# lixinghe1999/VRVQ

Hardware: AMD Instinct MI355X
Metric: audio-sec/s encode+RVQ+decode, 44.1 kHz batch-32, 1->8 MI355X; RVQ HBM GB/s (higher is better)
Workload: dtype f32; 1 GPU; DAC_VRVQ VBR 8 cb, level 1.0, 1-s clips, preprocess+encode+decode (z_q_is materialised); model=DAC_VRVQ base (8 cb), global_batch=32, clip_samples=44100, n_codebooks=8, parallelism=dp1 (replicas, no data-path collective)

## Files before the change

vrvq_amd/csrc/conv.hip:

```cpp
#include "common.h"
#include "conv_core.h"
#include "conv_x3.h"
#include <atomic>

namespace {

using namespace vrvq_conv;

template <int BM, int BN, int WM, int NW, int KS, bool X3, bool PH = false,
          bool PAIR = x3_pair<KS, BM, BN>(), bool SPLIT = false>
__global__ __launch_bounds__(64 * NW)
__attribute__((amdgpu_waves_per_eu(X3 && x3_stages<BM, BN>() == 1 ? 2 : 1)))
void conv_mfma_kernel(ConvArgs a) {
  using TC = TileCfg<BM, BN, WM, NW>;
  extern __shared__ __attribute__((aligned(16))) float smem[];
  int bid = blockIdx.x;
  int ks = 0;
  if (SPLIT) {
    ks = bid % a.ks_split;
    bid /= a.ks_split;
  }
  const int mt = bid % a.n_mt;
  bid /= a.n_mt;
  const int nt = bid % a.n_nt;
// ... 562 lines not shown
    const int kk = (int)(rk % k);
    const int ci = (int)(rk / k);
    wp[i] = co < cout ? w[((size_t)co * cin + ci) * k + kk] : 0.0f;
  }
}

__global__ void pack_convt1d_kernel(const float* __restrict__ w, int cin, int cout, int s,
                                    int cout_pad, float* __restrict__ wp) {
  const size_t total = (size_t)cin * 2 * cout_pad;
  for (size_t i = blockIdx.x * (size_t)blockDim.x + threadIdx.x; i < total;
       i += (size_t)gridDim.x * blockDim.x) {
    const int mm = (int)(i % cout_pad);
    const size_t rk = i / cout_pad;
    const int tap = (int)(rk % 2);
    const int ci = (int)(rk / 2);
    float v = 0.0f;
    if (mm < cout * s) {
      const int co = mm / s, r = mm - co * s;
      const int kk = tap == 1 ? r : r + s;
      v = w[((size_t)ci * cout + co) * (2 * s) + kk];
    }
    wp[i] = v;
  }
}

template <int KS>
__global__ void pack_x3_kernel(const float* __restrict__ wp, int cin, int m_pad,
                               u32x4* __restrict__ w3, size_t total) {
  using XC = X3Cfg<KS>;
  for (size_t i = blockIdx.x * (size_t)blockDim.x + threadIdx.x; i < total;
       i += (size_t)gridDim.x * blockDim.x) {
    const int m = (int)(i % m_pad);
    size_t r = i / m_pad;
    const int o = (int)(r % XC::NO2);
    r /= XC::NO2;
    const int plane = (int)(r % 3);
    const int chunk = (int)(r / 3);
    const int tap = o / XC::NC8, c8 = o - tap * XC::NC8;
    float v[8];
#pragma unroll
    for (int u = 0; u < 8; ++u) {
      const int ci = chunk * XC::CK + c8 * 8 + u;
      v[u] = (o < XC::NO && ci < cin) ? wp[((size_t)ci * KS + tap) * m_pad + m] : 0.0f;
    }
    unsigned h[4], mm[4], l[4];
#pragma unroll
    for (int u = 0; u < 4; ++u) split3x2(v[2 * u], v[2 * u + 1], h[u], mm[u], l[u]);
    w3[i] = plane == 0 ? u32x4{h[0], h[1], h[2], h[3]}
          : plane == 1 ? u32x4{mm[0], mm[1], mm[2], mm[3]} : u32x4{l[0], l[1], l[2], l[3]};
  }
}

static long long x3_size_u16(int cin, int k, int m_pad) {
  auto sz = [&](int ck, int no2) {
    return (long long)((cin + ck - 1) / ck) * 3 * no2 * m_pad * 8;
  };
  switch (k) {
    case 1: return sz(X3Cfg<1>::CK, X3Cfg<1>::NO2);
    case 2: return sz(X3Cfg<2>::CK, X3Cfg<2>::NO2);
    case 3: return sz(X3Cfg<3>::CK, X3Cfg<3>::NO2);
    case 7: return sz(X3Cfg<7>::CK, X3Cfg<7>::NO2);
    default: return -1;
  }
}

}

extern "C" int vrvq_x3_weight_size(int cin, int k, int cout_pad, long long* n_u16) {
  VRVQ_CHECK_ARG(n_u16 && cin > 0 && cout_pad > 0);
  const long long n = x3_size_u16(cin, k, cout_pad);
  if (n < 0) return VRVQ_ERR_UNSUPPORTED;
  *n_u16 = n;
  return 0;
}

extern "C" int vrvq_pack_x3_weight(const float* w_packed, int cin, int k, int cout_pad,
                                   uint16_t* w_x3, vrvq_stream_t stream) {
  VRVQ_CHECK_ARG(w_packed && w_x3 && cin > 0 && cout_pad > 0);
  const long long n = x3_size_u16(cin, k, cout_pad);
  if (n < 0) return VRVQ_ERR_UNSUPPORTED;
  const size_t total = (size_t)n / 8;
  const unsigned grid = (unsigned)((total + 255) / 256 < 65536 ? (total + 255) / 256 : 65536);
  u32x4* out = reinterpret_cast<u32x4*>(w_x3);
  hipStream_t st = as_stream(stream);
  switch (k) {
    case 1: hipLaunchKernelGGL(pack_x3_kernel<1>, dim3(grid), dim3(256), 0, st, w_packed, cin, cout_pad, out, total); break;
    case 2: hipLaunchKernelGGL(pack_x3_kernel<2>, dim3(grid), dim3(256), 0, st, w_packed, cin, cout_pad, out, total); break;
    case 3: hipLaunchKernelGGL(pack_x3_kernel<3>, dim3(grid), dim3(256), 0, st, w_packed, cin, cout_pad, out, total); break;
    default: hipLaunchKernelGGL(pack_x3_kernel<7>, dim3(grid), dim3(256), 0, st, w_packed, cin, cout_pad, out, total); break;
  }
  return vrvq_launch_status();
}

extern "C" int vrvq_conv1d(const float* x, int batch, int cin, int tin, const float* alpha,
                           const float* inv_alpha, const float* w_packed,
                           const uint16_t* w_x3, int cout,
                           int cout_pad, int k, int stride, int pad, int dil, const float* bias,
                           const float* residual, int epilogue, float* y, int tout,
                           const float* alpha_out, const float* inv_alpha_out, float* y_snake,
                           vrvq_stream_t stream) {
  return vrvq_conv1d_ws(x, batch, cin, tin, alpha, inv_alpha, w_packed, w_x3, cout, cout_pad, k,
                        stride, pad, dil, bias, residual, epilogue, y, tout, alpha_out,
                        inv_alpha_out, y_snake, nullptr, 0, stream);
}

extern "C" int vrvq_conv1d_workspace(int batch, int cin, int tin, int cout, int k, int stride,
                                     int pad, int dil, int x3, long long* bytes) {
  VRVQ_CHECK_ARG(bytes && batch > 0 && cin > 0 && tin > 0 && cout > 0 && k > 0 && stride > 0 &&
                 dil > 0 && pad >= 0);
  const long long tout = ((long long)tin + 2LL * pad - (long long)dil * (k - 1) - 1) / stride + 1;
  VRVQ_CHECK_ARG(tout > 0);
  int S = 0;
  if (stride > 1) {
    if (x3 && k == 2 * stride && (stride & (stride - 1)) == 0 && pad < stride)
      S = splitk_parts(cout, cin * stride, (int)tout, 2, true, false, true);
  } else {
    S = splitk_parts(cout, cin, (int)tout, k, false, false, x3 != 0);
  }
  *bytes = (long long)splitk_bytes(S, cout, (int)tout, batch);
  return 0;
}

extern "C" int vrvq_conv_last_launch(int out[5]) {
  VRVQ_CHECK_ARG(out);
  const unsigned v = g_last_launch.load(std::memory_order_relaxed);
  out[0] = (int)(v & 511);
  out[1] = (int)(v >> 9 & 511);
  out[2] = (int)(v >> 18 & 31);
  out[3] = (int)(v >> 23 & 3);
  out[4] = (int)(v >> 25 & 127);
  return 0;
}

namespace {


bool conv1d_geometry_ok(int batch, int cin, int tin, int cout, int cout_pad, int k, int stride,
                        int pad, int dil, int tout) {
  return batch > 0 && cin > 0 && tin > 0 && cout > 0 && k > 0 && stride > 0 && dil > 0 &&
         pad >= 0 && tout > 0 && cout_pad >= cout && cout_pad % 128 == 0 &&
         tout == ((long long)tin + 2LL * pad - (long long)dil * (k - 1) - 1) / stride + 1;
}

int run_conv1d(ConvArgs a, int batch, int cin, int tin, int cout, int cout_pad, int k, int stride,
               int pad, int dil, int tout, int epilogue, void* workspace, long long ws_bytes,
               hipStream_t st, ConvPlan* plan) {
  const bool proj = a.pj_part != nullptr;
  a.cin = cin; a.tin = tin; a.M = cout; a.m_pad = cout_pad; a.cout = cout;
  a.stride = stride; a.pad = pad; a.dil = dil; a.ng = tout; a.up = 0; a.up_pad = 0;
  a.ssh = 0;
  if (stride > 1 && (stride & (stride - 1)) == 0)
    while ((1 << a.ssh) < stride) ++a.ssh;
  a.ylen = tout; a.epi = epilogue;
  if (workspace != nullptr) {
    long long need = 0;
    const int rc = vrvq_conv1d_workspace(batch, cin, tin, cout, k, stride, pad, dil,
                                         a.w3 != nullptr, &need);
    if (rc) return rc;
    VRVQ_CHECK_ARG(ws_bytes >= need);
    if (need > 0) a.ks_part = static_cast<float*>(workspace);
  }
  if (a.w3 != nullptr && stride > 1) {
    if (k != 2 * stride || a.ssh == 0 || pad >= stride) return VRVQ_ERR_UNSUPPORTED;
    a.psh = a.ssh; a.ppad = pad; a.pcin = cin; a.ptin = tin;
    a.cin = cin * stride; a.tin = tout + 1;
    a.stride = 1; a.pad = 0; a.dil = 1; a.ssh = 0;
    return dispatch_ks(2, a, batch, st, plan);
  }
  if (!proj && cout <= SMALL_COUT && stride == 1 &&
      cin * k * (cout == 1 ? 1 : SMALL_COUT) <= SMALL_WMAX)
    return launch_small(a, batch, k, st, plan);
  if (!proj && cin == 1 && k == 7 && stride == 1 && dil == 1 && !a.alpha && cout % CI1_CG == 0 &&
      tout % 4 == 0) {
    const long long nblk =
        (long long)batch * ((tout + 256 * CI1_T - 1) / (256 * CI1_T)) * (cout / CI1_CG);
    if (nblk <= 0 || nblk > 0x7fffffffLL) return VRVQ_ERR_ARG;
    if (plan) *plan = ConvPlan{PATH_CIN1, 0, 0, 0, k, 0, 0};
    return launch_kernel(conv_cin1_stream_kernel<7>, nblk, 256, 0, st, a, plan != nullptr);
  }
  return dispatch_ks(k, a, batch, st, plan);
}

int run_conv_transpose1d(ConvArgs a, int batch, int cin, int tin, int cout, int cout_pad,
                         int stride, int pad, hipStream_t st, ConvPlan* plan) {
  VRVQ_CHECK_ARG(batch > 0 && cin > 0 && tin > 0 && cout > 0 && stride > 0);
  VRVQ_CHECK_ARG(pad >= 0 && pad < stride);
  VRVQ_CHECK_ARG(cout_pad >= cout * stride && cout_pad % 64 == 0);
  a.cin = cin; a.tin = tin; a.M = cout * stride; a.m_pad = cout_pad; a.cout = cout;
  a.stride = 1; a.pad = 1; a.dil = 1; a.ng = tin + 1; a.up = stride; a.up_pad = pad;
  a.ylen = (tin - 1) * stride - 2 * pad + 2 * stride;
  a.epi = VRVQ_EPI_NONE;
  return dispatch_ks(2, a, batch, st, plan);
}

}

extern "C" int vrvq_conv1d_ws(const float* x, int batch, int cin, int tin, const float* alpha,
                              const float* inv_alpha, const float* w_packed,
                              const uint16_t* w_x3, int cout, int cout_pad, int k, int stride,
                              int pad, int dil, const float* bias, const float* residual,
                              int epilogue, float* y, int tout, const float* alpha_out,
                              const float* inv_alpha_out, float* y_snake, void* workspace,
                              long long ws_bytes, vrvq_stream_t stream) {
  VRVQ_CHECK_ARG(x && w_packed && (y || y_snake));
  VRVQ_CHECK_ARG(y_snake == nullptr || (alpha_out && inv_alpha_out));
  VRVQ_CHECK_ARG(conv1d_geometry_ok(batch, cin, tin, cout, cout_pad, k, stride, pad, dil, tout));
  VRVQ_CHECK_ARG(alpha == nullptr || inv_alpha != nullptr);
  VRVQ_CHECK_ARG(epilogue >= 0 && epilogue <= 2);
  ConvArgs a{};
  a.x = x; a.alpha = alpha; a.inv_alpha = inv_alpha; a.w = w_packed;
  a.bias = bias; a.res = residual; a.y = y;
  a.alpha_o = alpha_out; a.inv_alpha_o = inv_alpha_out; a.ys = y_snake;
  a.w3 = reinterpret_cast<const unsigned*>(w_x3);
  return run_conv1d(a, batch, cin, tin, cout, cout_pad, k, stride, pad, dil, tout, epilogue,
                    workspace, ws_bytes, as_stream(stream), nullptr);
}

extern "C" int vrvq_conv1d_proj(const float* x, int batch, int cin, int tin, const float* alpha,
                                const float* inv_alpha, const float* w_packed,
                                const uint16_t* w_x3, int cout, int cout_pad, int k, int pad,
                                int dil, const float* bias, float* y, int tout,
                                const uint16_t* w3in, int nq, float* part, void* workspace,
                                long long ws_bytes, vrvq_stream_t stream) {
  VRVQ_CHECK_ARG(x && w_packed && w3in && part);
  VRVQ_CHECK_ARG(batch > 0 && cin > 0 && tin > 0 && cout > 0 && k > 0 && dil > 0 && pad >= 0 &&
                 tout > 0 && nq > 0);
  VRVQ_CHECK_ARG(cout_pad >= cout && cout_pad % 128 == 0);
  VRVQ_CHECK_ARG(alpha == nullptr || inv_alpha != nullptr);
  VRVQ_CHECK_ARG(((uintptr_t)part & 15) == 0 && ((uintptr_t)w3in & 15) == 0);
  if (cout != 1024 || nq > 32) return VRVQ_ERR_UNSUPPORTED;
  VRVQ_CHECK_ARG(conv1d_geometry_ok(batch, cin, tin, cout, cout_pad, k, 1, pad, dil, tout));
  VRVQ_CHECK_ARG((long long)batch * tout * nq * 8 * 8 < 0x7fffffffLL);
  ConvArgs a{};
  a.x = x; a.alpha = alpha; a.inv_alpha = inv_alpha; a.w = w_packed; a.bias = bias; a.y = y;
  a.w3 = reinterpret_cast<const unsigned*>(w_x3);
  a.pj_w3 = reinterpret_cast<const unsigned*>(w3in);
  a.pj_part = part;
  a.pj_nq = nq;
  a.pj_nf = batch * tout;
  return run_conv1d(a, batch, cin, tin, cout, cout_pad, k, 1, pad, dil, tout, VRVQ_EPI_NONE,
                    workspace, ws_bytes, as_stream(stream), nullptr);
}

extern "C" int vrvq_conv_transpose1d(const float* x, int batch, int cin, int tin,
                                     const float* alpha, const float* inv_alpha,
                                     const float* w_packed, int cout, int cout_pad, int stride,
                                     const float* bias, float* y, const float* alpha_out,
                                     const float* inv_alpha_out, float* y_snake,
                                     vrvq_stream_t stream) {
  return vrvq_conv_transpose1d_pad(x, batch, cin, tin, alpha, inv_alpha, w_packed, nullptr,
                                   cout, cout_pad, stride, (stride + 1) / 2, bias, y, alpha_out,
                                   inv_alpha_out, y_snake, stream);
}

extern "C" int vrvq_conv_transpose1d_pad(const float* x, int batch, int cin, int tin,
                                         const float* alpha, const float* inv_alpha,
                                         const float* w_packed, const uint16_t* w_x3,
                                         int cout, int cout_pad,
                                         int stride, int pad, const float* bias, float* y,
                                         const float* alpha_out, const float* inv_alpha_out,
                                         float* y_snake, vrvq_stream_t stream) {
  VRVQ_CHECK_ARG(x && w_packed && (y || y_snake));
  VRVQ_CHECK_ARG(y_snake == nullptr || (alpha_out && inv_alpha_out));
  VRVQ_CHECK_ARG(alpha == nullptr || inv_alpha != nullptr);
  ConvArgs a{};
  a.x = x; a.alpha = alpha; a.inv_alpha = inv_alpha; a.w = w_packed; a.bias = bias;
  a.res = nullptr; a.y = y;
  a.alpha_o = alpha_out; a.inv_alpha_o = inv_alpha_out; a.ys = y_snake;
  a.w3 = reinterpret_cast<const unsigned*>(w_x3);
  return run_conv_transpose1d(a, batch, cin, tin, cout, cout_pad, stride, pad, as_stream(stream),
                              nullptr);
}

extern "C" int vrvq_conv_plan(int kind, int batch, int cin, int tin, int cout, int k, int stride,
                              int pad, int dil, int has_x3, int has_workspace, int out[7]) {
  VRVQ_CHECK_ARG(out && kind >= VRVQ_PLAN_CONV && kind <= VRVQ_PLAN_CONV_TRANSPOSE);
  static float present[4];
  ConvArgs a{};
  a.w3 = has_x3 ? reinterpret_cast<const unsigned*>(present) : nullptr;
  void* ws = has_workspace ? present : nullptr;
  ConvPlan p{};
  int rc;
  if (kind == VRVQ_PLAN_CONV_TRANSPOSE) {
    VRVQ_CHECK_ARG(stride > 0 && k == 2 * stride && dil == 1);
    const long long rows = (long long)cout * stride, rt = 128 % stride == 0 ? 128 : 192;
    VRVQ_CHECK_ARG(cout > 0 && rows < 0x7fffff00LL);
    rc = run_conv_transpose1d(a, batch, cin, tin, cout, (int)((rows + rt - 1) / rt * rt), stride,
                              pad, nullptr, &p);
  } else {
    VRVQ_CHECK_ARG(cout > 0 && cout < 0x7fffff00 && k > 0 && stride > 0 && dil > 0 && tin > 0 &&
                   pad >= 0);
    const long long tout = ((long long)tin + 2LL * pad - (long long)dil * (k - 1) - 1) / stride + 1;
    const int cout_pad = (cout + 127) / 128 * 128;
    VRVQ_CHECK_ARG(tout > 0 && tout <= 0x7fffffffLL);
    VRVQ_CHECK_ARG(conv1d_geometry_ok(batch, cin, tin, cout, cout_pad, k, stride, pad, dil,
                                      (int)tout));
    if (kind == VRVQ_PLAN_PROJ) {
      VRVQ_CHECK_ARG(stride == 1);
      if (cout != 1024) return VRVQ_ERR_UNSUPPORTED;
      a.pj_part = present;
    }
    rc = run_conv1d(a, batch, cin, tin, cout, cout_pad, k, stride, pad, dil, (int)tout,
                    VRVQ_EPI_NONE, ws, 0x7fffffffffffffffLL, nullptr, &p);
  }
  if (rc) return rc;
  const int v[7] = {p.BM, p.BN, p.KS, p.x3, p.S, p.path, p.WM};
  for (int i = 0; i < 7; ++i) out[i] = v[i];
  return 0;
}

extern "C" int vrvq_pack_conv1d_weight(const float* w, int cout, int cin, int k, int cout_pad,
                                       float* w_packed, vrvq_stream_t stream) {
  VRVQ_CHECK_ARG(w && w_packed && cout > 0 && cin > 0 && k > 0 && cout_pad >= cout);
  const size_t total = (size_t)cin * k * cout_pad;
  const unsigned grid = (unsigned)((total + 255) / 256 < 65536 ? (total + 255) / 256 : 65536);
  hipLaunchKernelGGL(pack_conv1d_kernel, dim3(grid), dim3(256), 0, as_stream(stream), w, cout,
                     cin, k, cout_pad, w_packed);
  return vrvq_launch_status();
}

extern "C" int vrvq_pack_convt1d_weight(const float* w, int cin, int cout, int stride,
                                        int cout_pad, float* w_packed, vrvq_stream_t stream) {
  VRVQ_CHECK_ARG(w && w_packed && cout > 0 && cin > 0 && stride > 0 && cout_pad >= cout * stride);
  const size_t total = (size_t)cin * 2 * cout_pad;
  const unsigned grid = (unsigned)((total + 255) / 256 < 65536 ? (total + 255) / 256 : 65536);
  hipLaunchKernelGGL(pack_convt1d_kernel, dim3(grid), dim3(256), 0, as_stream(stream), w, cin,
                     cout, stride, cout_pad, w_packed);
  return vrvq_launch_status();
}
```

vrvq_amd/csrc/conv_ru.hip:

```cpp
#include "common.h"
#include "conv_core.h"
#include "conv_x3.h"

namespace {

using namespace vrvq_conv;

struct RuArgs {
  ConvArgs p1;
  ConvArgs p2;
  const float* b7;
  const float* alpha2;
  const float* inv_alpha2;
  const float* w1;
  const u32x4* w1x3;
  int C;
};

template <int BM, int BN>
constexpr bool ru_p2x3() { return BM * BN * 6 <= 80 * 1024; }
template <int BM, int BN, int WM>
constexpr bool ru_p2x3h() {
  return !ru_p2x3<BM, BN>() && WM == 2 && BM % 32 == 0 && BM * BN * 5 <= 80 * 1024;
}

template <int BM, int BN, int WM, int NW, bool X3>
__global__ __launch_bounds__(64 * NW)
__attribute__((amdgpu_waves_per_eu(X3 && x3_stages<BM, BN>() == 1 ? 2 : 1)))
void ru_fused_kernel(RuArgs ra) {
  using TC = TileCfg<BM, BN, WM, NW>;
  constexpr int RM = TC::RM, RN = TC::RN, TM = TC::TM, TN = TC::TN;
  constexpr int NS = BM / 2;
  constexpr int PF = 8;
  static_assert(NS % PF == 0, "phase-2 steps per group");
  extern __shared__ __attribute__((aligned(16))) float smem[];
  const ConvArgs& a = ra.p1;
  const int nt = blockIdx.x % a.n_nt;
  const int b = blockIdx.x / a.n_nt;
  const int n0 = nt * BN;
  const int C = ra.C;

  f32x16 acc[RM][RN];
#pragma unroll
  for (int i = 0; i < RM; ++i)
#pragma unroll
    for (int j = 0; j < RN; ++j)
#pragma unroll
      for (int r = 0; r < 16; ++r) acc[i][j][r] = 0.0f;
#ifdef VRVQ_X3_SB_ALL
  constexpr bool SB = true;
#else
  constexpr bool SB = BM == 96 || BM == 192 || BM == 128;
#endif
  if constexpr (X3) conv_mainloop_x3<BM, BN, WM, NW, 7, false, x3_pair<7, BM, BN>(), SB>(a, smem, acc, b, 0, n0);
  else conv_mainloop<BM, BN, WM, NW, 7>(a, smem, acc, b, 0, n0);

  const int tid = threadIdx.x, lane = tid & 63, wave = tid >> 6;
  const int wm = wave % WM, wn = wave / WM;
  const int lr = lane & 31, lh = lane >> 5;

  if constexpr (X3 && ru_p2x3<BM, BN>()) {
    if (ra.w1x3 != nullptr) {
      constexpr int NC8 = BM / 8;
      char* hsb = reinterpret_cast<char*>(smem);
#pragma unroll
      for (int i = 0; i < RM; ++i)
#pragma unroll
        for (int g = 0; g < 4; ++g) {
          const int row0 = wm * TM + i * 32 + 8 * g + 4 * lh;
          float bb[4], al[4], ia[4];
#pragma unroll
          for (int u = 0; u < 4; ++u) {
            const bool ok = row0 + u < C;
            bb[u] = ok ? ra.b7[row0 + u] : 0.0f;
            al[u] = ok ? ra.alpha2[row0 + u] : 0.0f;
            ia[u] = ok ? ra.inv_alpha2[row0 + u] : 0.0f;
          }
          const int c8 = (wm * TM + i * 32 + 8 * g) / 8;
#pragma unroll
          for (int j = 0; j < RN; ++j) {
            float v[4];
#pragma unroll
            for (int u = 0; u < 4; ++u) v[u] = acc[i][j][4 * g + u] + bb[u];
            snake_n<4>(v, al, ia);
#pragma unroll
            for (int u = 0; u < 4; ++u) v[u] = row0 + u < C ? v[u] : 0.0f;
            unsigned h[2], m[2], l[2];
            split3x2(v[0], v[1], h[0], m[0], l[0]);
            split3x2(v[2], v[3], h[1], m[1], l[1]);
            const int col = wn * TN + j * 32 + lr;
            const size_t off = ((size_t)c8 * BN + col) * 16 + lh * 8;
            typedef unsigned u32x2 __attribute__((ext_vector_type(2)));
            *reinterpret_cast<u32x2*>(hsb + off) = u32x2{h[0], h[1]};
            *reinterpret_cast<u32x2*>(hsb + (size_t)NC8 * BN * 16 + off) = u32x2{m[0], m[1]};
            *reinterpret_cast<u32x2*>(hsb + 2 * (size_t)NC8 * BN * 16 + off) = u32x2{l[0], l[1]};
          }
        }
      __syncthreads();
#pragma unroll
      for (int i = 0; i < RM; ++i)
#pragma unroll
        for (int j = 0; j < RN; ++j)
#pragma unroll
          for (int r = 0; r < 16; ++r) acc[i][j][r] = 0.0f;
      constexpr int NQ = BM / 16;
      const u32x4* hs = reinterpret_cast<const u32x4*>(hsb);
      auto lda = [&](int q, u32x4 (&av)[3][RM]) {
        const int o = 2 * q + lh;
        const int ch = o >> 2, oo = o & 3;
#pragma unroll
        for (int p = 0; p < 3; ++p)
#pragma unroll
          for (int i = 0; i < RM; ++i)
            av[p][i] = ra.w1x3[((size_t)(ch * 3 + p) * 4 + oo) * a.m_pad + wm * TM + i * 32 + lr];
      };
      u32x4 an[3][RM];
      lda(0, an);
#pragma unroll 2
      for (int q = 0; q < NQ; ++q) {
        u32x4 ac[3][RM], bv[3][RN];
#pragma unroll
        for (int p = 0; p < 3; ++p)
#pragma unroll
          for (int i = 0; i < RM; ++i) ac[p][i] = an[p][i];
        lda(min(q + 1, NQ - 1), an);
        const int o = 2 * q + lh;
#pragma unroll
        for (int p = 0; p < 3; ++p)
#pragma unroll
          for (int j = 0; j < RN; ++j) bv[p][j] = hs[((size_t)p * NC8 + o) * BN + wn * TN + j * 32 + lr];
#pragma unroll
        for (int i = 0; i < RM; ++i)
#pragma unroll
          for (int j = 0; j < RN; ++j) {
            f32x16 t = acc[i][j];
            t = mfma_bf16(ac[1][i], bv[1][j], t);
            t = mfma_bf16(ac[0][i], bv[2][j], t);
            t = mfma_bf16(ac[2][i], bv[0][j], t);
            t = mfma_bf16(ac[0][i], bv[1][j], t);
            t = mfma_bf16(ac[1][i], bv[0][j], t);
            acc[i][j] = mfma_bf16(ac[0][i], bv[0][j], t);
          }
      }
      __syncthreads();
      conv_epilogue<BM, BN, WM, NW>(ra.p2, smem, acc, b, 0, n0);
      return;
    }
  }

  if constexpr (X3 && ru_p2x3h<BM, BN, WM>()) {
    if (ra.w1x3 != nullptr) {
      constexpr int HC8 = BM / 16;
      constexpr int HQ = BM / 32;
      char* hsb = reinterpret_cast<char*>(smem);
      float* park = reinterpret_cast<float*>(hsb + (size_t)3 * HC8 * BN * 16);
      typedef unsigned u32x2 __attribute__((ext_vector_type(2)));
#pragma unroll
      for (int i = 0; i < RM; ++i)
#pragma unroll
        for (int g = 0; g < 4; ++g) {
          const int row0 = wm * TM + i * 32 + 8 * g + 4 * lh;
          float bb[4], al[4], ia[4];
#pragma unroll
          for (int u = 0; u < 4; ++u) {
            const bool ok = row0 + u < C;
            bb[u] = ok ? ra.b7[row0 + u] : 0.0f;
            al[u] = ok ? ra.alpha2[row0 + u] : 0.0f;
            ia[u] = ok ? ra.inv_alpha2[row0 + u] : 0.0f;
          }
#pragma unroll
          for (int j = 0; j < RN; ++j) {
            float v[4];
#pragma unroll
            for (int u = 0; u < 4; ++u) v[u] = acc[i][j][4 * g + u] + bb[u];
            snake_n<4>(v, al, ia);
#pragma unroll
            for (int u = 0; u < 4; ++u) v[u] = row0 + u < C ? v[u] : 0.0f;
            const int col = wn * TN + j * 32 + lr;
            if (row0 < BM / 2) {
              unsigned h[2], m[2], l[2];
              split3x2(v[0], v[1], h[0], m[0], l[0]);
              split3x2(v[2], v[3], h[1], m[1], l[1]);
              const size_t off = ((size_t)(row0 >> 3) * BN + col) * 16 + lh * 8;
              *reinterpret_cast<u32x2*>(hsb + off) = u32x2{h[0], h[1]};
              *reinterpret_cast<u32x2*>(hsb + (size_t)HC8 * BN * 16 + off) = u32x2{m[0], m[1]};
              *reinterpret_cast<u32x2*>(hsb + 2 * (size_t)HC8 * BN * 16 + off) = u32x2{l[0], l[1]};
            } else {
#pragma unroll
              for (int u = 0; u < 4; ++u) park[(row0 - BM / 2 + u) * BN + col] = v[u];
            }
          }
        }
      __syncthreads();
#pragma unroll
      for (int i = 0; i < RM; ++i)
#pragma unroll
        for (int j = 0; j < RN; ++j)
#pragma unroll
          for (int r = 0; r < 16; ++r) acc[i][j][r] = 0.0f;
      const u32x4* hs = reinterpret_cast<const u32x4*>(hsb);
      auto lda = [&](int q, u32x4 (&av)[3][RM]) {
        const int o = 2 * q + lh;
        const int ch = o >> 2, oo = o & 3;
#pragma unroll
        for (int p = 0; p < 3; ++p)
#pragma unroll
          for (int i = 0; i < RM; ++i)
            av[p][i] = ra.w1x3[((size_t)(ch * 3 + p) * 4 + oo) * a.m_pad + wm * TM + i * 32 + lr];
      };
      u32x4 an[3][RM];
      lda(0, an);
      auto steps = [&](int q0) {
#pragma unroll 2
        for (int q = q0; q < q0 + HQ; ++q) {
          u32x4 ac[3][RM], bv[3][RN];
#pragma unroll
          for (int p = 0; p < 3; ++p)
#pragma unroll
            for (int i = 0; i < RM; ++i) ac[p][i] = an[p][i];
          lda(min(q + 1, 2 * HQ - 1), an);
          const int o = 2 * (q - q0) + lh;
#pragma unroll
          for (int p = 0; p < 3; ++p)
#pragma unroll
            for (int j = 0; j < RN; ++j)
              bv[p][j] = hs[((size_t)p * HC8 + o) * BN + wn * TN + j * 32 + lr];
#pragma unroll
          for (int i = 0; i < RM; ++i)
#pragma unroll
            for (int j = 0; j < RN; ++j) {
              f32x16 t = acc[i][j];
              t = mfma_bf16(ac[1][i], bv[1][j], t);
              t = mfma_bf16(ac[0][i], bv[2][j], t);
              t = mfma_bf16(ac[2][i], bv[0][j], t);
              t = mfma_bf16(ac[0][i], bv[1][j], t);
              t = mfma_bf16(ac[1][i], bv[0][j], t);
              acc[i][j] = mfma_bf16(ac[0][i], bv[0][j], t);
            }
        }
      };
      steps(0);
      __syncthreads();
      for (int e = tid; e < HC8 * BN; e += 64 * NW) {
        const int c8 = e / BN, col = e - c8 * BN;
        float v[8];
#pragma unroll
        for (int u = 0; u < 8; ++u) v[u] = park[(c8 * 8 + u) * BN + col];
        unsigned h[4], m[4], l[4];
#pragma unroll
        for (int u = 0; u < 4; ++u) split3x2(v[2 * u], v[2 * u + 1], h[u], m[u], l[u]);
        u32x4* dst = reinterpret_cast<u32x4*>(hsb) + (size_t)c8 * BN + col;
        dst[0] = u32x4{h[0], h[1], h[2], h[3]};
        dst[(size_t)HC8 * BN] = u32x4{m[0], m[1], m[2], m[3]};
        dst[2 * (size_t)HC8 * BN] = u32x4{l[0], l[1], l[2], l[3]};
      }
      __syncthreads();
      steps(HQ);
      __syncthreads();
      conv_epilogue<BM, BN, WM, NW>(ra.p2, smem, acc, b, 0, n0);
      return;
    }
  }

  float* hs = smem;
#pragma unroll
  for (int i = 0; i < RM; ++i)
#pragma unroll
    for (int r = 0; r < 16; ++r) {
      const int row = wm * TM + i * 32 + (r & 3) + 8 * (r >> 2) + 4 * lh;
      const bool ok = row < C;
      const float bb = ok ? ra.b7[row] : 0.0f;
      const float al = ok ? ra.alpha2[row] : 0.0f, ia = ok ? ra.inv_alpha2[row] : 0.0f;
#pragma unroll
      for (int j = 0; j < RN; ++j) {
        const float v = acc[i][j][r] + bb;
        hs[row * BN + wn * TN + j * 32 + lr] = ok ? snake_act(v, al, ia) : 0.0f;
      }
    }
  __syncthreads();

#pragma unroll
  for (int i = 0; i < RM; ++i)
#pragma unroll
    for (int j = 0; j < RN; ++j)
#pragma unroll
      for (int r = 0; r < 16; ++r) acc[i][j][r] = 0.0f;
  const float* wa = ra.w1 + (size_t)lh * a.m_pad + wm * TM + lr;
  const float* hb = hs + lh * BN + wn * TN + lr;
  float an[PF][RM];
#pragma unroll
  for (int p = 0; p < PF; ++p)
#pragma unroll
    for (int i = 0; i < RM; ++i) an[p][i] = wa[(size_t)(2 * p) * a.m_pad + i * 32];
  for (int g = 0; g < NS; g += PF) {
    float ac[PF][RM];
#pragma unroll
    for (int p = 0; p < PF; ++p)
#pragma unroll
      for (int i = 0; i < RM; ++i) ac[p][i] = an[p][i];
    if (g + PF < NS) {
#pragma unroll
      for (int p = 0; p < PF; ++p)
#pragma unroll
        for (int i = 0; i < RM; ++i) an[p][i] = wa[(size_t)(2 * (g + PF + p)) * a.m_pad + i * 32];
    }
#pragma unroll
    for (int p = 0; p < PF; ++p) {
      float bv[RN];
#pragma unroll
      for (int j = 0; j < RN; ++j) bv[j] = hb[(2 * (g + p)) * BN + j * 32];
#pragma unroll
      for (int i = 0; i < RM; ++i)
#pragma unroll
        for (int j = 0; j < RN; ++j)
          acc[i][j] = __builtin_amdgcn_mfma_f32_32x32x2f32(ac[p][i], bv[j], acc[i][j], 0, 0, 0);
    }
  }
  __syncthreads();
  conv_epilogue<BM, BN, WM, NW>(ra.p2, smem, acc, b, 0, n0);
}

template <int BM, int BN, int WM, int NW>
int launch_ru(RuArgs ra, int batch, hipStream_t st) {
  constexpr int CK = ChunkCfg<7, BM, BN>::CK;
  ConvArgs& a = ra.p1;
  a.n_mt = 1;
  a.n_nt = (a.ng + BN - 1) / BN;
  ra.p2.n_mt = 1;
  ra.p2.n_nt = a.n_nt;
  if (a.m_pad < BM || ra.C > BM) return VRVQ_ERR_ARG;
  const int XW = (BN - 1) + 6 * a.dil + 1;
  const int XWP = (XW + 3) & ~3;
  if (XW > 64 * WinCfg<7, BN>::PER_ROW) return VRVQ_ERR_UNSUPPORTED;
  size_t lds = 2 * (size_t)(CK * 7 * BM + CK * XWP) * sizeof(float);
  const size_t hsz = (size_t)BM * BN * sizeof(float);
  const size_t epi = (size_t)BM * EpiCfg<BM, BN, NW / WM>::BNP * sizeof(float);
  if (lds < hsz) lds = hsz;
  if (lds < epi) lds = epi;
  const long long nblk = (long long)a.n_nt * batch;
  if (nblk <= 0 || nblk > 0x7fffffffLL) return VRVQ_ERR_ARG;
  if constexpr (BM <= 192) {
    size_t lx = x3_lds_bytes<7, BM, BN>(XW, a.cin);
    if (lx < hsz) lx = hsz;
    if (ru_p2x3<BM, BN>() && ra.w1x3 != nullptr && lx < (size_t)BM * BN * 6) lx = (size_t)BM * BN * 6;
    if (ru_p2x3h<BM, BN, WM>() && ra.w1x3 != nullptr && lx < (size_t)BM * BN * 5)
      lx = (size_t)BM * BN * 5;
    if (lx < epi) lx = epi;
    if (a.w3 != nullptr && XW <= (BN - 1) + 6 * 9 + 1 && lx <= 160 * 1024) {
      if (lx > 64 * 1024) {
        hipError_t e = hipFuncSetAttribute((const void*)ru_fused_kernel<BM, BN, WM, NW, true>,
                                           hipFuncAttributeMaxDynamicSharedMemorySize, (int)lx);
        if (e != hipSuccess) return (int)e;
      }
      hipLaunchKernelGGL((ru_fused_kernel<BM, BN, WM, NW, true>), dim3((unsigned)nblk),
                         dim3(64 * NW), lx, st, ra);
      return vrvq_launch_status();
    }
  }
  if (lds > 160 * 1024) return VRVQ_ERR_UNSUPPORTED;
  if (lds > 64 * 1024) {
    hipError_t e = hipFuncSetAttribute((const void*)ru_fused_kernel<BM, BN, WM, NW, false>,
                                       hipFuncAttributeMaxDynamicSharedMemorySize, (int)lds);
    if (e != hipSuccess) return (int)e;
  }
  hipLaunchKernelGGL((ru_fused_kernel<BM, BN, WM, NW, false>), dim3((unsigned)nblk),
                     dim3(64 * NW), lds, st, ra);
  return vrvq_launch_status();
}

}

extern "C" int vrvq_residual_unit(const float* x, const float* x_snk, int batch, int channels,
                                  int frames, int dil, const float* w7_packed,
                                  const uint16_t* w7_x3, const uint16_t* w1_x3,
                                  const float* b7,
                                  const float* alpha2, const float* inv_alpha2,
                                  const float* w1_packed, const float* b1, int cout_pad,
                                  float* y, const float* alpha_out, const float* inv_alpha_out,
                                  float* y_snake, vrvq_stream_t stream) {
  VRVQ_CHECK_ARG(x && x_snk && w7_packed && b7 && alpha2 && inv_alpha2 && w1_packed && b1);
  VRVQ_CHECK_ARG(y || y_snake);
  VRVQ_CHECK_ARG(y_snake == nullptr || (alpha_out && inv_alpha_out));
  VRVQ_CHECK_ARG(batch > 0 && channels > 0 && frames > 0 && dil >= 1 && dil <= 9);
  VRVQ_CHECK_ARG(cout_pad >= channels && cout_pad % 128 == 0);
  RuArgs ra{};
  ConvArgs& p = ra.p1;
  p.x = x_snk; p.alpha = nullptr; p.inv_alpha = nullptr; p.w = w7_packed; p.bias = nullptr;
  p.res = nullptr; p.y = nullptr; p.alpha_o = nullptr; p.inv_alpha_o = nullptr; p.ys = nullptr;
  p.cin = channels; p.tin = frames; p.M = channels; p.m_pad = cout_pad; p.cout = channels;
  p.stride = 1; p.pad = 3 * dil; p.dil = dil; p.ssh = 0; p.ng = frames; p.up = 0; p.up_pad = 0;
  p.ylen = frames; p.epi = VRVQ_EPI_NONE;
  p.w3 = reinterpret_cast<const unsigned*>(w7_x3);
  ConvArgs& q = ra.p2;
  q = p;
  q.bias = b1; q.res = x; q.y = y; q.alpha_o = alpha_out; q.inv_alpha_o = inv_alpha_out;
  q.ys = y_snake;
  ra.b7 = b7; ra.alpha2 = alpha2; ra.inv_alpha2 = inv_alpha2; ra.w1 = w1_packed;
  ra.w1x3 = w7_x3 != nullptr ? reinterpret_cast<const u32x4*>(w1_x3) : nullptr;
  ra.C = channels;
  hipStream_t st = as_stream(stream);
  switch (channels) {
    case 64: return launch_ru<64, 128, 2, 4>(ra, batch, st);
    case 96: return launch_ru<96, 128, 1, 4>(ra, batch, st);
    case 128: return launch_ru<128, 128, 2, 4>(ra, batch, st);
    case 192: return launch_ru<192, 64, 2, 4>(ra, batch, st);
    case 256: return launch_ru<256, 64, 2, 4>(ra, batch, st);
    default: return VRVQ_ERR_UNSUPPORTED;
  }
}
```

vrvq_amd/csrc/conv_x3.h:

```cpp
#pragma once
#include "conv_core.h"

typedef __bf16 bf16x8 __attribute__((ext_vector_type(8)));
typedef __bf16 bf16x2 __attribute__((ext_vector_type(2)));
typedef float f32x2 __attribute__((ext_vector_type(2)));
typedef unsigned u32x4 __attribute__((ext_vector_type(4)));

namespace vrvq_conv {

template <int BM, int BN>
constexpr int x3_stages() { return BM * BN <= 128 * 128 ? 1 : 2; }

template <int KS, int BM, int BN>
constexpr bool x3_pair() {
  return (KS == 7 && BM == 64 && BN == 256) ||
         (KS == 2 && BM <= 128 && (BN == 128 || BN == 32));
}

template <int KS, bool PAIR = false>
struct X3Cfg {
  static constexpr int CK = (PAIR ? 2 : 1) * (KS == 1 ? 32 : KS <= 3 ? 16 : 8);
  static constexpr int NC8 = CK / 8;
  static constexpr int NO = KS * NC8;
  static constexpr int NO2 = (NO + 1) & ~1;
  static constexpr int NSTEP = NO2 / 2;
};

__device__ __forceinline__ void split3x2(float v0, float v1, unsigned& h, unsigned& m,
                                         unsigned& l) {
  const f32x2 v = {v0, v1};
  const unsigned hu = __builtin_bit_cast(unsigned, __builtin_convertvector(v, bf16x2));
  const f32x2 hf = {__uint_as_float(hu << 16), __uint_as_float(hu & 0xffff0000u)};
  const f32x2 r = v - hf;
  const unsigned mu = __builtin_bit_cast(unsigned, __builtin_convertvector(r, bf16x2));
  const f32x2 mf = {__uint_as_float(mu << 16), __uint_as_float(mu & 0xffff0000u)};
  const f32x2 s = r - mf;
  h = hu;
  m = mu;
  l = __builtin_bit_cast(unsigned, __builtin_convertvector(s, bf16x2));
}

__device__ __forceinline__ f32x16 mfma_bf16(u32x4 a, u32x4 b, f32x16 c) {
  return __builtin_amdgcn_mfma_f32_32x32x16_bf16(__builtin_bit_cast(bf16x8, a),
                                                 __builtin_bit_cast(bf16x8, b), c, 0, 0, 0);
}

template <int KS, int BM, bool PAIR>
__host__ __device__ constexpr int x3_stage_w_bytes() {
  return PAIR ? 2 * 3 * X3Cfg<KS>::NO * BM * 16 : 3 * X3Cfg<KS>::NO2 * BM * 16;
}
__host__ __device__ inline int x3_xwp(int xw) { return (xw + 3) & ~3; }

template <int KS, int BM, bool PAIR, int NT>
struct X3W {
  static constexpr int TOTAL = x3_stage_w_bytes<KS, BM, PAIR>() / 16;
  static constexpr int WQ = (TOTAL + NT - 1) / NT;
};

template <int BM, int BN, int WM, int NW, int KS, bool PH = false,
          bool PAIR = x3_pair<KS, BM, BN>(), bool SB = false, bool XPF = false>
__device__ __forceinline__ void conv_mainloop_x3(
    const ConvArgs& a, float* smem,
    f32x16 (&acc)[TileCfg<BM, BN, WM, NW>::RM][TileCfg<BM, BN, WM, NW>::RN], int b, int m0,
    int n0, int kc0 = 0, int kc1 = 0x7fffffff) {
  using TC = TileCfg<BM, BN, WM, NW>;
  static_assert(!PAIR || ((KS == 7 || KS == 1) && !PH) || KS == 2,
                "pair chunks: k7 / k1 stride-1 windows, the 2-tap GEMMs");
  using XC = X3Cfg<KS, PAIR>;
  constexpr int NO2P = X3Cfg<KS>::NO2;
  constexpr int NOP = X3Cfg<KS>::NO;
  constexpr int NC8P = X3Cfg<KS>::NC8;
  static_assert(!PAIR || X3Cfg<KS, true>::NSTEP == NOP, "pair step q = packed octet q");
  constexpr int NT = TC::NT, RM = TC::RM, RN = TC::RN, TM = TC::TM, TN = TC::TN;
  constexpr int CK = XC::CK, NC8 = XC::NC8, NO = XC::NO, NO2 = XC::NO2, NSTEP = XC::NSTEP;
  constexpr int XW_MAX = (BN - 1) + (KS - 1) * (KS == 7 ? 9 : 1) + 1;
  constexpr int XI = (NC8 * XW_MAX + NT - 1) / NT;
  constexpr int WB = x3_stage_w_bytes<KS, BM, PAIR>();

  const int XW = (BN - 1) + (KS - 1) * a.dil + 1;
  const int XWP = x3_xwp(XW);
  const int STG = WB + 3 * NC8 * XWP * 16;
  constexpr int X3_STAGES = x3_stages<BM, BN>();
  const int tid = threadIdx.x, lane = tid & 63, wave = tid >> 6;
  const int wm = wave % WM, wn = wave / WM;
  const int lr = lane & 31, lh = lane >> 5;
  const u32x4* w3 = reinterpret_cast<const u32x4*>(a.w3);
  const int psh = PH ? a.psh : 0, pmask = (1 << psh) - 1, ppad = PH ? a.ppad : 0;
  const int ptin = PH ? a.ptin : a.tin;
  const float* xb = a.x + (size_t)b * (PH ? (size_t)a.pcin * a.ptin : (size_t)a.cin * a.tin);
  const int xbase = n0 - a.pad;
  const int nitems = NC8 * XW;
  char* sbase = reinterpret_cast<char*>(smem);


  constexpr int WQ = X3W<KS, BM, PAIR, NT>::WQ, WTOT = X3W<KS, BM, PAIR, NT>::TOTAL;
  u32x4 wr[WQ];
  auto load_w = [&](int chunk) {
#pragma unroll
    for (int r = 0; r < WQ; ++r) {
      const int u = min(tid + r * NT, WTOT - 1);
      if constexpr (PAIR) {
        const int hp = u / (NOP * BM), r2 = u - hp * (NOP * BM);
        const int po = r2 / BM, row = r2 - po * BM;
        const int half = hp / 3, pl = hp - half * 3;
        wr[r] = w3[(((size_t)(2 * chunk + half) * 3 + pl) * NO2P + po) * a.m_pad + m0 + row];
      } else {
        const int po = u / BM, row = u - po * BM;
        wr[r] = w3[((size_t)chunk * 3 * NO2 + po) * a.m_pad + m0 + row];
      }
    }
  };
  auto store_w = [&](char* stg) {
    u32x4* ws = reinterpret_cast<u32x4*>(stg);
#pragma unroll
    for (int r = 0; r < WQ; ++r)
      if (WTOT % NT == 0 || tid + r * NT < WTOT) ws[tid + r * NT] = wr[r];
  };
  float xr[XI][8];
  float* snl = reinterpret_cast<float*>(sbase + X3_STAGES * STG);
  auto load_x = [&](int ci0) {
#pragma unroll
    for (int it = 0; it < XI; ++it) {
      const int e = tid + it * NT;
      const int c8 = NC8 == 1 ? 0 : e / XW, pos = e - c8 * XW;
      const int tc = min(max(xbase + pos, 0), a.tin - 1);
      const int cb = ci0 + (e < nitems ? c8 : 0) * 8;
#pragma unroll
      for (int u = 0; u < 8; ++u) {
        const int cv = min(cb + u, a.cin - 1);
        if constexpr (PH) {
          const int tp = min(max((tc << psh) + (cv & pmask) - ppad, 0), ptin - 1);
          xr[it][u] = xb[(size_t)(cv >> psh) * ptin + tp];
        } else {
          xr[it][u] = xb[(size_t)cv * a.tin + tc];
        }
      }
    }
  };
  auto store_x = [&](char* stg, int ci0) {
    u32x4* xs = reinterpret_cast<u32x4*>(stg + WB);
    const bool sn = a.alpha != nullptr;
    constexpr int NU = NC8 == 1 ? 8 : 1;
    float alu[NU], iau[NU];
    if constexpr (NC8 == 1) {
      if (sn) {
#pragma unroll
        for (int u = 0; u < NU; ++u) {
          const int ci = PH ? min(ci0 + u, a.cin - 1) >> psh : min(ci0 + u, a.cin - 1);
          alu[u] = a.alpha[ci];
          iau[u] = a.inv_alpha[ci];
        }
      }
    }
#pragma unroll
    for (int it = 0; it < XI; ++it) {
      const int e = tid + it * NT;
      if (e >= nitems) continue;
      const int c8 = NC8 == 1 ? 0 : e / XW, pos = e - c8 * XW;
      const int t = xbase + pos;
      const bool okp = t >= 0 && t < a.tin;
      float v[8];
#pragma unroll
      for (int u = 0; u < 8; ++u) {
        const int cv = ci0 + c8 * 8 + u;
        bool ok = okp && cv < a.cin;
        if constexpr (PH) {
          const int tp = (t << psh) + (cv & pmask) - ppad;
          ok = ok && tp >= 0 && tp < ptin;
        }
        v[u] = ok ? xr[it][u] : 0.0f;
      }
      if (sn) {
        float al[8], ia[8];
#pragma unroll
        for (int u = 0; u < 8; ++u) {
          if constexpr (NC8 == 1) {
            al[u] = alu[u];
            ia[u] = iau[u];
          } else if constexpr (PAIR) {
            const int ci = min(ci0 + c8 * 8 + u, a.cin - 1) >> psh;
            al[u] = snl[ci];
            ia[u] = snl[(a.cin >> psh) + ci];
          } else {
            const int ci = PH ? min(ci0 + c8 * 8 + u, a.cin - 1) >> psh : min(ci0 + c8 * 8 + u, a.cin - 1);
            al[u] = a.alpha[ci];
            ia[u] = a.inv_alpha[ci];
          }
        }
        snake_n<8>(v, al, ia);
      }
      unsigned h[4], m[4], l[4];
#pragma unroll
      for (int u = 0; u < 4; ++u) split3x2(v[2 * u], v[2 * u + 1], h[u], m[u], l[u]);
      xs[(0 * NC8 + c8) * XWP + pos] = u32x4{h[0], h[1], h[2], h[3]};
      xs[(1 * NC8 + c8) * XWP + pos] = u32x4{m[0], m[1], m[2], m[3]};
      xs[(2 * NC8 + c8) * XWP + pos] = u32x4{l[0], l[1], l[2], l[3]};
    }
  };

  const int nchunks = min((a.cin + CK - 1) / CK, kc1);
  const int col = wn * TN + lr;
  auto rd_at = [&](const u32x4* ws, const u32x4* xs, int q, u32x4 (&av)[3][RM], u32x4 (&bv)[3][RN]) {
    const int o = 2 * q + lh;
    const int tap = PAIR ? q / NC8P : o < NO ? o / NC8 : 0;
    const int c8 = PAIR ? lh * NC8P + q % NC8P : o - (o / NC8) * NC8;
    const int wo = PAIR ? lh * 3 * NOP + q : o;
#pragma unroll
    for (int p = 0; p < 3; ++p)
#pragma unroll
      for (int i = 0; i < RM; ++i)
        av[p][i] = ws[(p * (PAIR ? NOP : NO2) + wo) * BM + wm * TM + i * 32 + lr];
    const int xo = c8 * XWP + col + tap * a.dil;
#pragma unroll
    for (int p = 0; p < 3; ++p)
#pragma unroll
      for (int j = 0; j < RN; ++j) bv[p][j] = xs[p * NC8 * XWP + xo + j * 32];
  };
  auto mma_at = [&](const u32x4 (&av)[3][RM], const u32x4 (&bv)[3][RN]) {
#pragma unroll
    for (int i = 0; i < RM; ++i)
#pragma unroll
      for (int j = 0; j < RN; ++j) {
        f32x16 t = acc[i][j];
        t = mfma_bf16(av[1][i], bv[1][j], t);
        t = mfma_bf16(av[0][i], bv[2][j], t);
        t = mfma_bf16(av[2][i], bv[0][j], t);
        t = mfma_bf16(av[0][i], bv[1][j], t);
        t = mfma_bf16(av[1][i], bv[0][j], t);
        acc[i][j] = mfma_bf16(av[0][i], bv[0][j], t);
      }
  };
  auto chunk_mma = [&](const u32x4* ws, const u32x4* xs) {
    if constexpr (SB) {
#pragma unroll
      for (int q = 0; q < NSTEP; ++q) {
        u32x4 a0[3][RM], b0[3][RN];
        rd_at(ws, xs, q, a0, b0);
        mma_at(a0, b0);
      }
      return;
    }
    u32x4 a0[3][RM], b0[3][RN], a1[3][RM], b1[3][RN];
    rd_at(ws, xs, 0, a0, b0);
#pragma unroll
    for (int q = 0; q < NSTEP; q += 2) {
      if (q + 1 < NSTEP) rd_at(ws, xs, q + 1, a1, b1);
      __builtin_amdgcn_sched_barrier(0);
      mma_at(a0, b0);
      __builtin_amdgcn_sched_barrier(0);
      if (q + 2 < NSTEP) rd_at(ws, xs, q + 2, a0, b0);
      __builtin_amdgcn_sched_barrier(0);
      if (q + 1 < NSTEP) mma_at(a1, b1);
      __builtin_amdgcn_sched_barrier(0);
    }
  };
  if constexpr (PAIR) {
    if (a.alpha != nullptr) {
      const int nsc = a.cin >> psh;
      for (int c = tid; c < nsc; c += NT) {
        snl[c] = a.alpha[c];
        snl[nsc + c] = a.inv_alpha[c];
      }
      __syncthreads();
    }
  }
  int cur = 0;
  load_w(kc0);
  load_x(kc0 * CK);
  store_w(sbase);
  store_x(sbase, kc0 * CK);
  __syncthreads();
  for (int c = kc0; c < nchunks; ++c) {
    const int cn = min(c + 1, nchunks - 1);
    char* nxt = sbase + (cur ^ (X3_STAGES - 1)) * STG;
    if constexpr (X3_STAGES == 2) {
      load_w(cn);
      load_x(cn * CK);
      __builtin_amdgcn_sched_barrier(0);
    } else if constexpr (XPF) {
      load_x(cn * CK);
      __builtin_amdgcn_sched_barrier(0);
    }
    chunk_mma(reinterpret_cast<const u32x4*>(sbase + cur * STG),
              reinterpret_cast<const u32x4*>(sbase + cur * STG + WB));
    if constexpr (X3_STAGES == 1) {
      __syncthreads();
      if (c + 1 < nchunks) {
        load_w(cn);
        if constexpr (!XPF) load_x(cn * CK);
        __builtin_amdgcn_sched_barrier(0);
        store_w(nxt);
        store_x(nxt, cn * CK);
      }
    } else {
      store_w(nxt);
      store_x(nxt, cn * CK);
    }
    __syncthreads();
    cur ^= X3_STAGES - 1;
  }
}

template <int KS, int BM, int BN, bool PAIR = x3_pair<KS, BM, BN>()>
inline size_t x3_lds_bytes(int xw, int cin) {
  const size_t xb = 3 * (size_t)X3Cfg<KS, PAIR>::NC8 * x3_xwp(xw) * 16;
  const size_t snake = PAIR ? 2 * (size_t)cin * sizeof(float) : 0;
  return x3_stages<BM, BN>() * ((size_t)x3_stage_w_bytes<KS, BM, PAIR>() + xb) + snake;
}

}
```

Baseline: 765.5 audio-sec/s.

## Precompute per-thread 32-bit gather offsets and advance chunk base pointers in x3 loaders

```diff
diff --git a/vrvq_amd/csrc/conv.hip b/vrvq_amd/csrc/conv.hip
--- a/vrvq_amd/csrc/conv.hip
+++ b/vrvq_amd/csrc/conv.hip
@@ -738,6 +738,7 @@
   if (stride > 1 && (stride & (stride - 1)) == 0)
     while ((1 << a.ssh) < stride) ++a.ssh;
   a.ylen = tout; a.epi = epilogue;
+  if (a.w3 != nullptr && !x3_offsets_fit(tin, cout_pad)) return VRVQ_ERR_UNSUPPORTED;
   if (workspace != nullptr) {
     long long need = 0;
     const int rc = vrvq_conv1d_workspace(batch, cin, tin, cout, k, stride, pad, dil,
@@ -772,6 +773,7 @@
   VRVQ_CHECK_ARG(batch > 0 && cin > 0 && tin > 0 && cout > 0 && stride > 0);
   VRVQ_CHECK_ARG(pad >= 0 && pad < stride);
   VRVQ_CHECK_ARG(cout_pad >= cout * stride && cout_pad % 64 == 0);
+  if (a.w3 != nullptr && !x3_offsets_fit(tin, cout_pad)) return VRVQ_ERR_UNSUPPORTED;
   a.cin = cin; a.tin = tin; a.M = cout * stride; a.m_pad = cout_pad; a.cout = cout;
   a.stride = 1; a.pad = 1; a.dil = 1; a.ng = tin + 1; a.up = stride; a.up_pad = pad;
   a.ylen = (tin - 1) * stride - 2 * pad + 2 * stride;
diff --git a/vrvq_amd/csrc/conv_ru.hip b/vrvq_amd/csrc/conv_ru.hip
--- a/vrvq_amd/csrc/conv_ru.hip
+++ b/vrvq_amd/csrc/conv_ru.hip
@@ -105,14 +105,16 @@
           for (int r = 0; r < 16; ++r) acc[i][j][r] = 0.0f;
       constexpr int NQ = BM / 16;
       const u32x4* hs = reinterpret_cast<const u32x4*>(hsb);
+      const unsigned wlo = ((unsigned)lh * (unsigned)a.m_pad + (unsigned)(wm * TM + lr)) * 16u;
       auto lda = [&](int q, u32x4 (&av)[3][RM]) {
-        const int o = 2 * q + lh;
-        const int ch = o >> 2, oo = o & 3;
+        const u32x4* wq = ra.w1x3 + (size_t)((q >> 1) * 12 + 2 * (q & 1)) * a.m_pad;
+        const unsigned wl = x3_opaque(wlo);
 #pragma unroll
         for (int p = 0; p < 3; ++p)
 #pragma unroll
           for (int i = 0; i < RM; ++i)
-            av[p][i] = ra.w1x3[((size_t)(ch * 3 + p) * 4 + oo) * a.m_pad + wm * TM + i * 32 + lr];
+            av[p][i] = *reinterpret_cast<const u32x4*>(
+                reinterpret_cast<const char*>(wq + (size_t)(p * 4) * a.m_pad + i * 32) + wl);
       };
       u32x4 an[3][RM];
       lda(0, an);
@@ -383,6 +385,7 @@
   VRVQ_CHECK_ARG(y_snake == nullptr || (alpha_out && inv_alpha_out));
   VRVQ_CHECK_ARG(batch > 0 && channels > 0 && frames > 0 && dil >= 1 && dil <= 9);
   VRVQ_CHECK_ARG(cout_pad >= channels && cout_pad % 128 == 0);
+  if (w7_x3 != nullptr && !x3_offsets_fit(frames, cout_pad)) return VRVQ_ERR_UNSUPPORTED;
   RuArgs ra{};
   ConvArgs& p = ra.p1;
   p.x = x_snk; p.alpha = nullptr; p.inv_alpha = nullptr; p.w = w7_packed; p.bias = nullptr;
diff --git a/vrvq_amd/csrc/conv_x3.h b/vrvq_amd/csrc/conv_x3.h
--- a/vrvq_amd/csrc/conv_x3.h
+++ b/vrvq_amd/csrc/conv_x3.h
@@ -38,6 +38,11 @@
   h = hu;
   m = mu;
   l = __builtin_bit_cast(unsigned, __builtin_convertvector(s, bf16x2));
+}
+
+__device__ __forceinline__ unsigned x3_opaque(unsigned v) {
+  asm volatile("" : "+v"(v));
+  return v;
 }
 
 __device__ __forceinline__ f32x16 mfma_bf16(u32x4 a, u32x4 b, f32x16 c) {
@@ -94,19 +99,47 @@
 
 
   constexpr int WQ = X3W<KS, BM, PAIR, NT>::WQ, WTOT = X3W<KS, BM, PAIR, NT>::TOTAL;
+  auto w_slot = [](int g) {
+    if constexpr (PAIR && NOP != NO2P) return (g / NOP) * NO2P + g % NOP;
+    else return g;
+  };
+  constexpr bool WUNI = BM % 64 == 0;
+  static_assert(WUNI || (BM % 32 == 0 && NT % 32 == 0 && !(PAIR && NOP != NO2P)), "W offsets");
+  constexpr int WP = BM == 32 ? 1 : BM / 32;
+  static_assert(WUNI || (NT * WP) % BM == 0, "W offsets: period");
+  constexpr bool WLAST = WTOT % NT != 0;
+  constexpr int WNV = WUNI ? 1 : (WQ < WP ? WQ : WP) + 1;
+  const int wv = __builtin_amdgcn_readfirstlane(tid >> 6);
+  const unsigned lane16 = (unsigned)lane * 16u;
+  unsigned wvo[WNV];
+  if constexpr (!WUNI) {
+    auto w_off = [&](int u) {
+      const int g = u / BM, row = u - g * BM;
+      return ((unsigned)g * (unsigned)a.m_pad + (unsigned)row) * 16u;
+    };
+#pragma unroll
+    for (int r = 0; r < WNV - 1; ++r) wvo[r] = w_off(tid + r * NT);
+    wvo[WNV - 1] = w_off(min(tid + (WQ - 1) * NT, WTOT - 1));
+  }
+  const size_t wstride = (size_t)(PAIR ? 2 : 1) * 3 * NO2P * a.m_pad;
+  const u32x4* wc = w3 + (size_t)kc0 * wstride + m0;
   u32x4 wr[WQ];
-  auto load_w = [&](int chunk) {
+  auto load_w = [&]() {
+    unsigned vo[WNV];
+#pragma unroll
+    for (int i = 0; i < WNV; ++i) vo[i] = x3_opaque(WUNI ? lane16 : wvo[i]);
 #pragma unroll
     for (int r = 0; r < WQ; ++r) {
-      const int u = min(tid + r * NT, WTOT - 1);
-      if constexpr (PAIR) {
-        const int hp = u / (NOP * BM), r2 = u - hp * (NOP * BM);
-        const int po = r2 / BM, row = r2 - po * BM;
-        const int half = hp / 3, pl = hp - half * 3;
-        wr[r] = w3[(((size_t)(2 * chunk + half) * 3 + pl) * NO2P + po) * a.m_pad + m0 + row];
+      if constexpr (WUNI) {
+        const int un = min(wv + r * (NT / 64), WTOT / 64 - 1);
+        const int g = (un * 64) / BM, rowb = un * 64 - g * BM;
+        const u32x4* ws = wc + ((unsigned)w_slot(g) * (unsigned)a.m_pad + (unsigned)rowb);
+        wr[r] = *reinterpret_cast<const u32x4*>(reinterpret_cast<const char*>(ws) + vo[0]);
+      } else if (WLAST && r == WQ - 1) {
+        wr[r] = *reinterpret_cast<const u32x4*>(reinterpret_cast<const char*>(wc) + vo[WNV - 1]);
       } else {
-        const int po = u / BM, row = u - po * BM;
-        wr[r] = w3[((size_t)chunk * 3 * NO2 + po) * a.m_pad + m0 + row];
+        const u32x4* ws = wc + (unsigned)((r / WP) * (NT * WP / BM)) * (unsigned)a.m_pad;
+        wr[r] = *reinterpret_cast<const u32x4*>(reinterpret_cast<const char*>(ws) + vo[r % WP]);
       }
     }
   };
@@ -117,29 +150,71 @@
       if (WTOT % NT == 0 || tid + r * NT < WTOT) ws[tid + r * NT] = wr[r];
   };
   float xr[XI][8];
+  unsigned xvo[XI];
+  int xso[XI], xts[PH ? XI : 1];
+  bool xokp[XI];
+#pragma unroll
+  for (int it = 0; it < XI; ++it) {
+    const int e = tid + it * NT;
+    const int c8 = NC8 == 1 ? 0 : e / XW, pos = e - c8 * XW;
+    const int t = xbase + pos;
+    const int tc = min(max(t, 0), a.tin - 1);
+    const int c8v = e < nitems ? c8 : 0;
+    if constexpr (PH) {
+      xts[it] = (tc << psh) - ppad;
+      xvo[it] = (unsigned)(c8v * (8 >> psh)) * (unsigned)ptin * 4u;
+    } else {
+      xvo[it] = ((unsigned)(c8v * 8) * (unsigned)a.tin + (unsigned)tc) * 4u;
+    }
+    xso[it] = e < nitems ? c8 * XWP + pos : -1;
+    xokp[it] = t >= 0 && t < a.tin;
+  }
+  const size_t xstride = (size_t)(CK >> psh) * ptin;
+  const float* xc = xb + (size_t)kc0 * xstride;
   float* snl = reinterpret_cast<float*>(sbase + X3_STAGES * STG);
   auto load_x = [&](int ci0) {
+    if (!PAIR && ci0 + CK > a.cin) {
+#pragma unroll
+      for (int it = 0; it < XI; ++it) {
+        const int e = tid + it * NT;
+        const int c8 = NC8 == 1 ? 0 : e / XW, pos = e - c8 * XW;
+        const int tc = min(max(xbase + pos, 0), a.tin - 1);
+        const int cb = ci0 + (e < nitems ? c8 : 0) * 8;
+#pragma unroll
+        for (int u = 0; u < 8; ++u) {
+          const int cv = min(cb + u, a.cin - 1);
+          if constexpr (PH) {
+            const int tp = min(max((tc << psh) + (cv & pmask) - ppad, 0), ptin - 1);
+            xr[it][u] = xb[(size_t)(cv >> psh) * ptin + tp];
+          } else {
+            xr[it][u] = xb[(size_t)cv * a.tin + tc];
+          }
+        }
+      }
+      return;
+    }
+    int ts[PH ? XI : 1];
+    unsigned vo[XI];
 #pragma unroll
     for (int it = 0; it < XI; ++it) {
-      const int e = tid + it * NT;
-      const int c8 = NC8 == 1 ? 0 : e / XW, pos = e - c8 * XW;
-      const int tc = min(max(xbase + pos, 0), a.tin - 1);
-      const int cb = ci0 + (e < nitems ? c8 : 0) * 8;
-#pragma unroll
-      for (int u = 0; u < 8; ++u) {
-        const int cv = min(cb + u, a.cin - 1);
-        if constexpr (PH) {
-          const int tp = min(max((tc << psh) + (cv & pmask) - ppad, 0), ptin - 1);
-          xr[it][u] = xb[(size_t)(cv >> psh) * ptin + tp];
-        } else {
-          xr[it][u] = xb[(size_t)cv * a.tin + tc];
-        }
+      vo[it] = x3_opaque(xvo[it]);
+      if constexpr (PH) ts[it] = (int)x3_opaque((unsigned)xts[it]);
+    }
+#pragma unroll
+    for (int u = 0; u < 8; ++u) {
+      const char* xu = reinterpret_cast<const char*>(xc + (size_t)(u >> psh) * ptin);
+#pragma unroll
+      for (int it = 0; it < XI; ++it) {
+        unsigned o = vo[it];
+        if constexpr (PH) o += (unsigned)min(max(ts[it] + (u & pmask), 0), ptin - 1) * 4u;
+        xr[it][u] = *reinterpret_cast<const float*>(xu + o);
       }
     }
   };
   auto store_x = [&](char* stg, int ci0) {
     u32x4* xs = reinterpret_cast<u32x4*>(stg + WB);
     const bool sn = a.alpha != nullptr;
+    const bool ragged = !PAIR && ci0 + CK > a.cin;
     constexpr int NU = NC8 == 1 ? 8 : 1;
     float alu[NU], iau[NU];
     if constexpr (NC8 == 1) {
@@ -154,20 +229,15 @@
     }
 #pragma unroll
     for (int it = 0; it < XI; ++it) {
-      const int e = tid + it * NT;
-      if (e >= nitems) continue;
-      const int c8 = NC8 == 1 ? 0 : e / XW, pos = e - c8 * XW;
-      const int t = xbase + pos;
-      const bool okp = t >= 0 && t < a.tin;
+      if (xso[it] < 0) continue;
+      const int c8 = NC8 == 1 ? 0 : (tid + it * NT) / XW;
+      const int ts = PH ? (int)x3_opaque((unsigned)xts[it]) : 0;
       float v[8];
 #pragma unroll
       for (int u = 0; u < 8; ++u) {
-        const int cv = ci0 + c8 * 8 + u;
-        bool ok = okp && cv < a.cin;
-        if constexpr (PH) {
-          const int tp = (t << psh) + (cv & pmask) - ppad;
-          ok = ok && tp >= 0 && tp < ptin;
-        }
+        bool ok = xokp[it];
+        if (ragged) ok = ok && ci0 + c8 * 8 + u < a.cin;
+        if constexpr (PH) ok = ok && (unsigned)(ts + (u & pmask)) < (unsigned)ptin;
         v[u] = ok ? xr[it][u] : 0.0f;
       }
       if (sn) {
@@ -192,9 +262,9 @@
       unsigned h[4], m[4], l[4];
 #pragma unroll
       for (int u = 0; u < 4; ++u) split3x2(v[2 * u], v[2 * u + 1], h[u], m[u], l[u]);
-      xs[(0 * NC8 + c8) * XWP + pos] = u32x4{h[0], h[1], h[2], h[3]};
-      xs[(1 * NC8 + c8) * XWP + pos] = u32x4{m[0], m[1], m[2], m[3]};
-      xs[(2 * NC8 + c8) * XWP + pos] = u32x4{l[0], l[1], l[2], l[3]};
+      xs[0 * NC8 * XWP + xso[it]] = u32x4{h[0], h[1], h[2], h[3]};
+      xs[1 * NC8 * XWP + xso[it]] = u32x4{m[0], m[1], m[2], m[3]};
+      xs[2 * NC8 * XWP + xso[it]] = u32x4{l[0], l[1], l[2], l[3]};
     }
   };
 
@@ -265,16 +335,18 @@
     }
   }
   int cur = 0;
-  load_w(kc0);
+  load_w();
   load_x(kc0 * CK);
   store_w(sbase);
   store_x(sbase, kc0 * CK);
   __syncthreads();
   for (int c = kc0; c < nchunks; ++c) {
     const int cn = min(c + 1, nchunks - 1);
+    wc += c + 1 < nchunks ? wstride : 0;
+    xc += c + 1 < nchunks ? xstride : 0;
     char* nxt = sbase + (cur ^ (X3_STAGES - 1)) * STG;
     if constexpr (X3_STAGES == 2) {
-      load_w(cn);
+      load_w();
       load_x(cn * CK);
       __builtin_amdgcn_sched_barrier(0);
     } else if constexpr (XPF) {
@@ -286,7 +358,7 @@
     if constexpr (X3_STAGES == 1) {
       __syncthreads();
       if (c + 1 < nchunks) {
-        load_w(cn);
+        load_w();
         if constexpr (!XPF) load_x(cn * CK);
         __builtin_amdgcn_sched_barrier(0);
         store_w(nxt);
@@ -299,6 +371,10 @@
     __syncthreads();
     cur ^= X3_STAGES - 1;
   }
+}
+
+inline bool x3_offsets_fit(long long tin, long long m_pad) {
+  return 32 * tin * 4 <= 0x7fffffffLL && 49 * m_pad * 16 <= 0x7fffffffLL;
 }
 
 template <int KS, int BM, int BN, bool PAIR = x3_pair<KS, BM, BN>()>
```

Measured after the change: 784.4 audio-sec/s, median of 6. 2.5% higher.
